# NguyenThaiHoc1/CustomKnowledgeGraphEmbedding

Measured on AMD Instinct MI355X. Metric: scored (pos+neg) triples/sec, WN18RR InterHT d=1000 n_neg=256, 1/2/4/8 GPU, higher is better.
Workload: dtype f32; 1 GPU; WN18RR InterHT d=1000 -de -tr gamma=24 n_neg=256 bz=512; global_batch=512, n_neg=256, hidden_dim=1000, score_function=InterHT, parallelism=single

## Files before the change

### customknowledgegraphembedding_amd/_lib.py

```python
from __future__ import annotations

import ctypes
import os
import threading

_HERE = os.path.dirname(os.path.abspath(__file__))
LIB_PATH = os.environ.get("KGE_HIP_LIB", os.path.join(_HERE, "libkge_hip.so"))

FN_IDS = {
    "TransE": 0,
    "DistMult": 1,
    "ComplEx": 2,
    "RotatE": 3,
    "InterHT": 4,
    "pRotatE": 5,
}
HEAD_BATCH, TAIL_BATCH, SINGLE = 0, 1, 3

_c_i64 = ctypes.c_int64
_c_f = ctypes.c_float
_c_p = ctypes.c_void_p
_c_i = ctypes.c_int


# ... 33 lines not shown
        _c_i,
        [_c_i, _c_i, _c_p, _c_i64, _c_i64, _c_p, _c_i64, _c_i64, _c_i64, _c_p, _c_p, _c_i64,
         _c_i64, _c_i64, _c_i64, _c_f, _c_f, _c_f, _c_p, _c_i64, _c_p, _c_p],
    ),
    "kge_step_forward_ex": (
        _c_i,
        [_c_i, _c_i, _c_p, _c_i64, _c_i64, _c_p, _c_i64, _c_i64, _c_i64, _c_p, _c_p, _c_i64,
         _c_i64, _c_i64, _c_i64, _c_f, _c_f, _c_f, _c_f, _c_i, _c_p, _c_i64, _c_p, _c_p, _c_p, _c_p, _c_p, _c_p],
    ),
    "kge_step_plan_size": (_c_i64, [_c_i, _c_i64, _c_i64, _c_i64, _c_i64, _c_i64, _c_i64, _c_i64, _c_i64]),
    "kge_step_plan": (
        _c_i, [_c_i, _c_i, _c_i64, _c_i64, _c_i64, _c_i64, _c_i64, _c_p, _c_p, _c_i64, _c_i64, _c_i64, _c_i64, _c_p,
               _c_p]),
    "kge_step_forward_planned": (
        _c_i,
        [_c_i, _c_i, _c_p, _c_i64, _c_i64, _c_p, _c_i64, _c_i64, _c_i64, _c_i64, _c_i64, _c_i64, _c_f, _c_f, _c_f,
         _c_f, _c_i, _c_p, _c_p, _c_p, _c_i64, _c_i, _c_p, _c_p, _c_i64, _c_p, _c_p, _c_p, _c_p],
    ),
    "kge_step_planner_create": (
        _c_i, [_c_p, _c_i, _c_p, _c_i64, _c_i64, _c_p, _c_i64, _c_i64, _c_i64, _c_i64, _c_i64, _c_i64, _c_f, _c_f, _c_f,
               _c_f, _c_i, _c_p, _c_p, _c_i64, _c_p]),
    "kge_step_planner_set_modulus": (_c_i, [_c_p, _c_f]),
    "kge_step_planner_set_sweep": (_c_i, [_c_p, _c_i]),
    "kge_step_planner_plan": (_c_i, [_c_p, _c_p, _c_p, _c_i64, _c_i]),
    "kge_step_planner_step": (_c_i, [_c_p, _c_p, _c_p, _c_i64, _c_i, _c_p, _c_p, _c_p, _c_p]),
    "kge_step_planner_destroy": (_c_i, [_c_p]),
    "kge_step_finish": (
        _c_i,
        [_c_i, _c_p, _c_i64, _c_i64, _c_p, _c_i64, _c_i64, _c_i64, _c_p, _c_i64, _c_i64,
         _c_f, _c_f, _c_f, _c_p, _c_i64, _c_i64, _c_f, _c_i, _c_p, _c_p, _c_p, _c_p],
    ),
    "kge_score_sharded": (
        _c_i,
        [_c_i, _c_i, _c_p, _c_i64, _c_p, _c_i64, _c_i64, _c_i64, _c_p, _c_i64, _c_i64, _c_i64,
         _c_p, _c_p, _c_i64, _c_i64, _c_i64, _c_i64, _c_f, _c_f, _c_f, _c_p, _c_i64, _c_p],
    ),
    "kge_gather_rows": (
        _c_i, [_c_p, _c_i64, _c_i64, _c_i64, _c_p, _c_i64, _c_i64, _c_i64, _c_p, _c_i64, _c_p]),
    "kge_build_id": (ctypes.c_char_p, []),
    "kge_source_hash": (ctypes.c_char_p, []),
    "kge_shard_plan": (
        _c_i, [_c_p, _c_p, _c_i64, _c_i64, _c_i64, _c_i64, _c_i, _c_i, _c_i, _c_i, _c_i, _c_p, _c_p, _c_p, _c_p, _c_p,
               _c_p, _c_p, _c_p]),
    "kge_shard_gather_queries": (
        _c_i, [_c_p, _c_i64, _c_i64, _c_i64, _c_p, _c_i64, _c_i, _c_i, _c_i64, _c_i, _c_i, _c_i, _c_i, _c_p, _c_p,
               _c_p, _c_p, _c_p, _c_p]),
# ... 189 lines not shown
```

### customknowledgegraphembedding_amd/csrc/kge_abi.hip

```cpp
#include <string.h>

#include <algorithm>
#include <cmath>

#include <string>

#include "kge_device.h"
#include "kge_scan.h"

namespace kge_impl {
namespace {

__global__ __launch_bounds__(kBlock) void neg_reduce_kernel(const float* __restrict__ s, int64_t B, int64_t N,
                                                            int64_t ld, float T, int adversarial,
                                                            float* __restrict__ out) {
    const int64_t b = (int64_t)blockIdx.x * kWavesPerBlock + (threadIdx.x >> 6);
    if (b >= B) return;
    const int lane = threadIdx.x & 63;
    const float res = row_reduce_fast(s + b * ld, N, T, adversarial, lane);
    if (lane == 0) out[b] = res;
}

__global__ __launch_bounds__(kBlock) void neg_rows_kernel(ScoreParams p) {
    const int64_t b = (int64_t)blockIdx.x * kWavesPerBlock + (threadIdx.x >> 6);
// ... 508 lines not shown

int step_order(int64_t nentity, int64_t N, const kge_forms* forms = nullptr) {
    const int forced = forms ? forms->step_order : -1;
    if (nentity >= (int64_t)8 << 25) return 0;
    if (forced >= 0 && forced <= 2) return forced;
    return N >= 128 ? 2 : 0;
}
bool use_xcd_order(int64_t nentity, int64_t N, const kge_forms* forms = nullptr) {
    return step_order(nentity, N, forms) != 0;
}

int tile_plan(int fn, ScoreParams& p, const kge_forms* forms = nullptr) {
    int V = 1, G = 1;
    if (pick_vg(p, V, G)) return 0;
    if (G > kFwdGradMaxG || p.N + 1 > 65536 || p.c_rows <= 0) return 0;
    const int64_t opb = (int64_t)G * kWave * V * 4;
    int64_t P2 = 0;
    if (fn == KGE_INTERHT && p.B <= kTileSortMaxB) {
        P2 = kWave;
        while (P2 < p.B) P2 <<= 1;
    }
    const int64_t row_bytes = (int64_t)p.D * 4 * (is_split(fn) ? 2 : 1);
    p.tile_waves = row_bytes >= 4096 ? 12 : 16;
    const int fw = forms ? forms->tile_waves : 0;
    if (fw == 8 || fw == 12 || fw == 16) p.tile_waves = fw;
    const int64_t NT = (int64_t)p.tile_waves * kWave;
    const int64_t qrow = tile_nq(fn) * opb + 8 + 8 + 8 + 4, lrow = (p.N + 1) * 4;
    const int64_t fixed = kTileBuckets * 4 + 16;
    const int64_t sort_ints = P2 ? (kTileSortMaxB + NT - 1) / NT * p.tile_waves * kTileSortRel : 0;
    auto lds = [&](int64_t R, int64_t QS) { return R * qrow + QS * opb + fixed + std::max(R * lrow, sort_ints * 4); };
    int64_t R = kTileMaxRows;
    if (forms && forms->tile_rows > 0) R = std::min<int64_t>(R, forms->tile_rows);
    while (R >= 1 && lds(R, 0) > kTileLdsMax) --R;
    if (R < 1) return 0;
    int64_t QS = 0;
    if (fn == KGE_INTERHT)
        while (QS < R && lds(R, QS + 1) <= kTileLdsMax) ++QS;
    if (forms && forms->tile_q2slots >= 0) QS = std::min<int64_t>(QS, forms->tile_q2slots);
#ifdef KGE_PROFILING_KNOBS
    p.tile_dry = getenv("KGE_TILE_DRY") ? std::max(1, atoi(getenv("KGE_TILE_DRY"))) : 0;
    if (getenv("KGE_TILE_NOSORT")) P2 = 0;
#endif
    p.tile_rows = (int)R;
    p.tile_q2slots = (int)QS;
    p.tile_sort = (int)P2;
    p.tile_lds = (int)lds(R, QS);
    return 1;
}

int planned_tile_params(int fn, int64_t nentity, int64_t ent_ld, int64_t nrelation, int64_t rel_ld, int64_t rel_off,
                        int64_t B, int64_t N, int64_t D, ScoreParams& p) {
    if (B <= 0 || N <= 0 || D <= 0 || nentity <= 0 || nentity >= ((int64_t)1 << 31) || B >= ((int64_t)1 << 31))
        return 0;
    const float* tab = reinterpret_cast<const float*>((uintptr_t)4096);
    fill_indexed(p, fn, KGE_TAIL_BATCH, tab, nentity, ent_ld, tab, nrelation, rel_ld, rel_off, nullptr, nullptr, 0, B,
                 N, D, 0.f, 1.f, 0.f);
    return tile_plan(fn, p) ? p.tile_rows : 0;
}

PlanArgs plan_args(const ScoreParams& tp, int mode, int64_t nentity, int64_t nrelation, const int64_t* pos,
                   const int64_t* neg, int64_t neg_ld, int64_t B, int64_t N, void* plan) {
    PlanArgs a;
    a.pos = pos;
    a.neg = neg;
    a.neg_ld = neg_ld;
    a.B = B;
    a.N = N;
    a.nent = nentity;
    a.nrel = nrelation;
    a.mode = mode;
    a.R = tp.tile_rows;
    a.sort = tp.tile_sort != 0;
    a.plan = reinterpret_cast<int*>(plan);
    return a;
}

}

int set_error(int code, const char* msg) { return fail(code, msg); }
}
// ... 135 lines not shown
        return fail(KGE_EINVAL, "kge_step_plan needs a negative mode (0 or 1)");
    if (B <= 0 || N <= 0 || D <= 0) return fail(KGE_EINVAL, "bad shape (B, N, D)");
    if (!pos || !neg || !plan) return fail(KGE_EINVAL, "null pointer");
    if (!aligned(plan, 16)) return fail(KGE_EINVAL, "the plan must be 16-B aligned");
    ScoreParams tp;
    if (!planned_tile_params(fn, nentity, ent_ld, nrelation, rel_ld, rel_off, B, N, D, tp))
        return fail(KGE_ENOTSUP, "the tile form does not apply to this shape (kge_step_plan_size is 0)");
    const PlanArgs a = plan_args(tp, mode, nentity, nrelation, pos, neg, neg_ld, B, N, plan);
    const unsigned groups = (unsigned)plan_groups(B, tp.tile_rows);
    if (tp.tile_waves == 16)
        hipLaunchKernelGGL(tile_plan_kernel<16>, dim3(groups), dim3(16 * kWave), plan_lds_ints(16 * kWave) * 4,
                           (hipStream_t)stream, a);
    else
        hipLaunchKernelGGL(tile_plan_kernel<12>, dim3(groups), dim3(12 * kWave), plan_lds_ints(12 * kWave) * 4,
                           (hipStream_t)stream, a);
    return check_launch("kge_step_plan");
}

static int step_forward_planned(int fn, int mode, const float* ent, int64_t nentity, int64_t ent_ld, const float* rel,
                                int64_t nrelation, int64_t rel_ld, int64_t rel_off, int64_t B, int64_t N, int64_t D,
                                float gamma, float emb_range, float modulus, float temperature, int adversarial,
                                const void* plan, const int64_t* next_pos, const int64_t* next_neg,
                                int64_t next_neg_ld, int next_mode, void* next_plan, float* neg_scores, int64_t ns_ld,
                                float* out_neg, float* pos_scores, float* out_pos, int reverse, void* stream);

int kge_step_forward_planned(int fn, int mode, const float* ent, int64_t nentity, int64_t ent_ld, const float* rel,
                             int64_t nrelation, int64_t rel_ld, int64_t rel_off, int64_t B, int64_t N, int64_t D,
                             float gamma, float emb_range, float modulus, float temperature, int adversarial,
                             const void* plan, const int64_t* next_pos, const int64_t* next_neg, int64_t next_neg_ld,
                             int next_mode, void* next_plan, float* neg_scores, int64_t ns_ld, float* out_neg,
                             float* pos_scores, float* out_pos, void* stream) {
    return step_forward_planned(fn, mode, ent, nentity, ent_ld, rel, nrelation, rel_ld, rel_off, B, N, D, gamma,
                                emb_range, modulus, temperature, adversarial, plan, next_pos, next_neg, next_neg_ld,
                                next_mode, next_plan, neg_scores, ns_ld, out_neg, pos_scores, out_pos, 0, stream);
}

static int step_forward_planned(int fn, int mode, const float* ent, int64_t nentity, int64_t ent_ld, const float* rel,
                                int64_t nrelation, int64_t rel_ld, int64_t rel_off, int64_t B, int64_t N, int64_t D,
                                float gamma, float emb_range, float modulus, float temperature, int adversarial,
                                const void* plan, const int64_t* next_pos, const int64_t* next_neg,
                                int64_t next_neg_ld, int next_mode, void* next_plan, float* neg_scores, int64_t ns_ld,
                                float* out_neg, float* pos_scores, float* out_pos, int reverse, void* stream) {
    int rc = check_fn_mode(fn, mode);
    if (rc) return rc;
    if (mode == KGE_SINGLE) return fail(KGE_EINVAL, "kge_step_forward_planned needs a negative mode (0 or 1)");
    if (B <= 0 || N <= 0 || D <= 0) return fail(KGE_EINVAL, "bad shape (B, N, D)");
    if (!ent || !rel || !plan || !neg_scores || !out_neg || !out_pos) return fail(KGE_EINVAL, "null pointer");
    if (next_plan) {
        if (next_mode != KGE_HEAD_BATCH && next_mode != KGE_TAIL_BATCH)
            return fail(KGE_EINVAL, "the next batch needs a negative mode (0 or 1)");
        if (!next_pos || !next_neg) return fail(KGE_EINVAL, "next_plan needs next_pos and next_neg");
        if (next_plan == plan) return fail(KGE_EINVAL, "next_plan must not be the plan this step reads");
        if (!aligned(next_plan, 16)) return fail(KGE_EINVAL, "the plan must be 16-B aligned");
    }
    if (!aligned(plan, 16)) return fail(KGE_EINVAL, "the plan must be 16-B aligned");
    ScoreParams tp;
    const int R = planned_tile_params(fn, nentity, ent_ld, nrelation, rel_ld, rel_off, B, N, D, tp);
    ScoreParams p;
    fill_indexed(p, fn, mode, ent, nentity, ent_ld, rel, nrelation, rel_ld, rel_off, nullptr, nullptr, 0, B, N, D,
                 gamma, emb_range, modulus);
    if (!R || !tile_plan(fn, p) || p.tile_rows != R)
        return fail(KGE_ENOTSUP, "the tile form does not apply to these tables (unaligned rows, or "
                                 "kge_step_plan_size is 0): use kge_step_forward");
    p.out = neg_scores;
    p.out_ld = ns_ld;
    p.pos_base = nullptr;
    p.temperature = temperature;
    p.adversarial = adversarial;
    p.out_neg = out_neg;
    p.out_pos_raw = pos_scores;
    p.out_pos_ls = out_pos;
    p.tile_pos = 1;
    p.tile_rev = reverse;
    p.tile_plan = reinterpret_cast<const int*>(plan);
    if (next_plan) {
        p.tile_next = plan_args(tp, next_mode, nentity, nrelation, next_pos, next_neg, next_neg_ld, B, N, next_plan);
        p.tile_lds = std::max(p.tile_lds, plan_lds_ints(p.tile_waves * kWave) * 4);
    }
    rc = run_score(fn, mode, p, KIND_STEP_FWD_TILE, stream);
    if (rc) return rc;
    const int64_t blocks = (B + kWavesPerBlock - 1) / kWavesPerBlock;
    hipLaunchKernelGGL(neg_rows_kernel, dim3((unsigned)blocks), dim3(kBlock), 0, (hipStream_t)stream, p);
    return check_launch("kge_step_forward_planned row reductions");
}

struct kge_step_planner {
    int fn = 0, adversarial = 1;
    const float* ent = nullptr;
    const float* rel = nullptr;
    int64_t nentity = 0, ent_ld = 0, nrelation = 0, rel_ld = 0, rel_off = 0, B = 0, N = 0, D = 0;
    float gamma = 0.f, emb_range = 0.f, modulus = 0.f, temperature = 1.f;
    void* plans[2] = {nullptr, nullptr};
    int cur = -1;
    int mode = 0;
    int sweep = 1;
    int64_t steps = 0;
    void* stream = nullptr;
};

int kge_step_planner_create(kge_step_planner** out, int fn, const float* ent, int64_t nentity, int64_t ent_ld,
                            const float* rel, int64_t nrelation, int64_t rel_ld, int64_t rel_off, int64_t B, int64_t N,
                            int64_t D, float gamma, float emb_range, float modulus, float temperature, int adversarial,
                            void* plan0, void* plan1, int64_t plan_bytes, void* stream) {
    if (!out) return fail(KGE_EINVAL, "kge_step_planner_create: null pointer");
    *out = nullptr;
    const int64_t need = kge_step_plan_size(fn, nentity, ent_ld, nrelation, rel_ld, rel_off, B, N, D);
    if (need <= 0) return fail(KGE_ENOTSUP, "kge_step_planner_create: the tile form does not apply to this shape");
    if (!ent || !rel || !plan0 || !plan1 || plan0 == plan1) return fail(KGE_EINVAL, "kge_step_planner_create: bad pointers");
    if (plan_bytes < need || !aligned(plan0, 16) || !aligned(plan1, 16))
        return fail(KGE_EINVAL, "kge_step_planner_create: plan buffers too small or not 16-B aligned");
    kge_step_planner* sp = new kge_step_planner;
    sp->fn = fn;
    sp->ent = ent;
    sp->nentity = nentity;
    sp->ent_ld = ent_ld;
    sp->rel = rel;
    sp->nrelation = nrelation;
    sp->rel_ld = rel_ld;
    sp->rel_off = rel_off;
    sp->B = B;
    sp->N = N;
    sp->D = D;
    sp->gamma = gamma;
    sp->emb_range = emb_range;
    sp->modulus = modulus;
    sp->temperature = temperature;
    sp->adversarial = adversarial;
    sp->plans[0] = plan0;
    sp->plans[1] = plan1;
    sp->stream = stream;
    *out = sp;
    return ok();
}

int kge_step_planner_set_modulus(kge_step_planner* sp, float modulus) {
    if (!sp) return fail(KGE_EINVAL, "kge_step_planner_set_modulus: null pointer");
    sp->modulus = modulus;
    return ok();
}

int kge_step_planner_set_sweep(kge_step_planner* sp, int alternate) {
    if (!sp) return fail(KGE_EINVAL, "kge_step_planner_set_sweep: null pointer");
    if (alternate != 0 && alternate != 1) return fail(KGE_EINVAL, "kge_step_planner_set_sweep: 0 or 1");
    sp->sweep = alternate;
    return ok();
}

int kge_step_planner_plan(kge_step_planner* sp, const int64_t* pos, const int64_t* neg, int64_t neg_ld, int mode) {
    if (!sp) return fail(KGE_EINVAL, "kge_step_planner_plan: null pointer");
    const int buf = sp->cur < 0 ? 0 : sp->cur;
    const int rc = kge_step_plan(sp->fn, mode, sp->nentity, sp->ent_ld, sp->nrelation, sp->rel_ld, sp->rel_off, pos, neg,
                                 neg_ld, sp->B, sp->N, sp->D, sp->plans[buf], sp->stream);
    if (rc) return rc;
    sp->cur = buf;
    sp->mode = mode;
    return ok();
}

int kge_step_planner_step(kge_step_planner* sp, const int64_t* next_pos, const int64_t* next_neg, int64_t next_neg_ld,
                          int next_mode, float* neg_scores, float* out_neg, float* pos_scores, float* out_pos) {
    if (!sp) return fail(KGE_EINVAL, "kge_step_planner_step: null pointer");
    if (sp->cur < 0) return fail(KGE_EINVAL, "kge_step_planner_step: no batch planned (kge_step_planner_plan first)");
    const bool nxt = next_pos && next_neg;
    const int rc = step_forward_planned(
        sp->fn, sp->mode, sp->ent, sp->nentity, sp->ent_ld, sp->rel, sp->nrelation, sp->rel_ld, sp->rel_off, sp->B,
        sp->N, sp->D, sp->gamma, sp->emb_range, sp->modulus, sp->temperature, sp->adversarial, sp->plans[sp->cur],
        next_pos, next_neg, next_neg_ld, next_mode, nxt ? sp->plans[1 - sp->cur] : nullptr, neg_scores, sp->N, out_neg,
        pos_scores, out_pos, sp->sweep ? (int)(sp->steps & 1) : 0, sp->stream);
    if (rc) return rc;
    ++sp->steps;
    if (nxt) {
        sp->cur = 1 - sp->cur;
        sp->mode = next_mode;
    } else {
        sp->cur = -1;
    }
    return ok();
}

int kge_step_planner_destroy(kge_step_planner* sp) {
    delete sp;
    return ok();
}

int kge_score_sharded(int fn, int mode, const float* qent, int64_t q_ld, const float* rel, int64_t nrelation,
                      int64_t rel_ld, int64_t rel_off, const float* shard, int64_t shard_rows, int64_t shard_ld,
                      int64_t shard_lo, const int64_t* pos, const int64_t* neg, int64_t neg_ld, int64_t B, int64_t N,
                      int64_t D, float gamma, float emb_range, float modulus, float* scores, int64_t scores_ld,
                      void* stream) {
    int rc = check_fn_mode(fn, mode);
    if (rc) return rc;
// ... 1028 lines not shown
```

### customknowledgegraphembedding_amd/csrc/kge_device.h

```cpp
#pragma once

#include <math.h>

#include <type_traits>

#include "kge_internal.h"

namespace kge_impl {

template <int V>
struct alignas(4 * V) vecf {
    float a[V];
};

template <int V>
__device__ __forceinline__ vecf<V> vzero() {
    vecf<V> r;
#pragma unroll
    for (int i = 0; i < V; ++i) r.a[i] = 0.f;
    return r;
}

template <int V>
__device__ __forceinline__ vecf<V> vload(const float* p, bool ok) {
// ... 881 lines not shown
    }
    auto chk = [](int64_t id, int64_t n) { return (id >= 0 && id < n) ? (int)id : -1; };
    if (t < R)
        reinterpret_cast<int4*>(a.plan + kPlanHdr)[(int64_t)g * R + t] =
            t < nr ? make_int4(brow[t], chk(ph, a.nent), chk(pr, a.nrel), chk(pt, a.nent)) : make_int4(-1, -1, -1, -1);
    if (g == 0 && t == 0) {
        int* h = a.plan;
        h[0] = kPlanMagic;
        h[1] = (int)a.B;
        h[2] = (int)a.N;
        h[3] = a.mode;
        h[4] = R;
        h[5] = (int)a.nent;
        h[6] = a.sort;
    }
}

template <int NWV>
__global__ __launch_bounds__(NWV * kWave) void tile_plan_kernel(PlanArgs a) {
    extern __shared__ __attribute__((aligned(16))) unsigned char plan_smem[];
    tile_plan_group<NWV>(a, (int)blockIdx.x, reinterpret_cast<int*>(plan_smem));
}

template <int FN, bool CH, int V, int G, int NWV>
__global__ __launch_bounds__(NWV * kWave) void step_fwd_tile_kernel(ScoreParams p) {
    extern __shared__ __attribute__((aligned(16))) unsigned char tile_smem[];
    constexpr int NQ = tile_nq(FN);
    constexpr int W = G * kWave;
    constexpr int NT = NWV * kWave;
    const int R = p.tile_rows, QS = p.tile_q2slots;
    vecf<V>* qimg = reinterpret_cast<vecf<V>*>(tile_smem);
    vecf<V>* q2img = qimg + (size_t)R * NQ * W;
    int64_t* rrow = reinterpret_cast<int64_t*>(q2img + (size_t)QS * W);
    int64_t* brow = rrow + R;
    int64_t* qid = brow + R;
    int* q2slot = reinterpret_cast<int*>(qid + R);
    int* hist = q2slot + R;
    int* cntp = hist + kTileBuckets;
    int* list = cntp + 4;
    const int t = threadIdx.x, lane = t & 63, w = t >> 6;
    if (p.tile_next.plan && (int)blockIdx.x >= p.tile_blocks) {
        tile_plan_group<NWV>(p.tile_next, (int)blockIdx.x - p.tile_blocks, reinterpret_cast<int*>(tile_smem));
        return;
    }
    const int x = (int)(blockIdx.x & 7);
    const int gi = (int)(blockIdx.x >> 3);
    const int64_t g0 = (int64_t)gi * R;
    const int nr = (int)min<int64_t>(R, p.B - g0);
// ... 233 lines not shown
        }
        if (lane == kWave - 1) cntp[0] = incl;
    }
    __syncthreads();
    if (pl) {
    } else if (in_regs) {
#pragma unroll
        for (int u = 0; u < TPI; ++u)
            if (wbk[u] >= 0) list[hist[wbk[u]] + wrk[u]] = wcd[u];
    } else {
        for (int64_t f = t; f < nf; f += NT) {
            int bk, code;
            if (item(f, bk, code)) list[atomicAdd(&hist[bk], 1)] = code;
        }
    }
    __syncthreads();
    const int cnt = pl ? pcnt : cntp[0];

    if (p.tile_dry) return;
    struct Item {
        Cand<FN, V, G> c;
        vecf<V> q2[FN == KGE_INTERHT ? G : 1];
    };
    for (int c0 = w; c0 < cnt; c0 += NT) {
        const int nc = min(kWave, (cnt - c0 + NWV - 1) / NWV);
        int code = 0;
        int64_t my_id = 0;
        if (lane < nc) {
            const int ci = p.tile_rev ? cnt - 1 - (c0 + NWV * lane) : c0 + NWV * lane;
            if (pl) {
                const int2 e = plist[plo + ci];
                code = e.y;
                my_id = e.x;
            } else {
                code = list[ci];
                const int r = code >> 16, n = code & 0xFFFF;
                const int64_t b = brow[r];
                my_id = n < p.N ? p.c_idx[b * p.c_stride + n] : p.pos_base[b * 3 + 2];
            }
        }
        auto load = [&](Item& it, int j) {
            bool ok;
            it.c.load(cand_row(p, readlane64(my_id, j), ok), ok, p.D, lane);
            if constexpr (FN == KGE_INTERHT) {
                const int r = __builtin_amdgcn_readlane(code, j) >> 16;
                const int sl = q2slot[r];
// ... 4 lines not shown
                    const int64_t ri = rrow[r];
                    const rsrc_t sr = make_rsrc(p.rel + (ri >= 0 ? ri : 0) * p.r_ld + p.r_off,
                                                ri >= 0 ? (uint32_t)p.D * 4u : 0u);
#pragma unroll
                    for (int k = 0; k < G; ++k) it.q2[k] = bload<V>(sr, goff<V>(lane, k));
                }
            }
        };
        auto score = [&](const Item& it, int j) -> float {
            const int cj = __builtin_amdgcn_readlane(code, j);
            const int r = cj >> 16, n = cj & 0xFFFF;
            const vecf<V>* qr = qimg + (size_t)r * NQ * W;
            (void)n;
            if constexpr (FN == KGE_INTERHT) {
                TileQueryIH<V, G> q{{qr, lane}, {qr + W, lane}, {}};
#pragma unroll
                for (int k = 0; k < G; ++k) q.q2[k] = it.q2[k];
                return cand_score<FN, CH, V, G>(it.c, q, p);
            } else {
                const LdsQuery<V> q{{qr, lane}, {qr + (NQ > 1 ? W : 0), lane}, {qr, lane}};
                return cand_score<FN, CH, V, G>(it.c, q, p);
            }
        };
        float my_score = 0.f;
        {
            Item x0, x1;
            load(x0, 0);
            for (int j = 0; j < nc; j += 2) {
                if (j + 1 < nc) load(x1, j + 1);
                float s = score(x0, j);
                if (lane == j) my_score = s;
                if (j + 1 < nc) {
                    if (j + 2 < nc) load(x0, j + 2);
                    s = score(x1, j + 1);
                    if (lane == j + 1) my_score = s;
                }
            }
        }
        if (lane < nc) {
            const int r = code >> 16, n = code & 0xFFFF;
            const int64_t b = brow[r];
            if (n < p.N) {
                p.out[b * p.out_ld + n] = my_score;
            } else {
                if (p.out_pos_raw) p.out_pos_raw[b] = my_score;
                p.out_pos_ls[b] = log_sigmoid(my_score);
            }
        }
    }
    if constexpr (CH) {
        if (!p.tile_pos) return;
        for (int r = w; r < nr; r += NWV) {
            const int64_t b = brow[r];
            const int4 pm = pl ? pmeta[r] : make_int4(0, 0, 0, 0);
            const int64_t tt = pl ? pm.w : p.pos_base[b * 3 + 2], row = tt - p.c_base;
            const bool valid = row >= 0 && row < p.c_rows;
            if (valid ? (row < e_lo || row >= e_hi) : x != 0) continue;
            Query<FN, false, V, G> qp;
            const int64_t hi = pl ? pm.y : p.pos_base[b * 3], rj = pl ? pm.z : p.pos_base[b * 3 + 1];
            const bool hok = hi >= 0 && hi < p.q_rows, rjok = rj >= 0 && rj < p.r_rows;
            qp.build(p.qent + (hok ? hi : 0) * p.q_ld, hok, p.rel + (rjok ? rj : 0) * p.r_ld + p.r_off, rjok, p.D,
                     lane, p);
            bool ok;
            Cand<FN, V, G> c;
            c.load(cand_row(p, tt, ok), ok, p.D, lane);
            const float s = cand_score<FN, false, V, G>(c, qp, p);
            if (lane == 0) {
                if (p.out_pos_raw) p.out_pos_raw[b] = s;
                p.out_pos_ls[b] = log_sigmoid(s);
            }
        }
    }
// ... 1763 lines not shown
                    adam_update(pp.a[i], gr.a[i], mm[h][gg].a[i], vv[h][gg].a[i], p.adam.b1, p.adam.b2, p.adam.eps,
                                p.adam.alpha, p.adam.step_size, p.adam.bc2_sqrt, p.adam.keras);
                sstore(sp, goffs[gg], pp);
                sstore(sm, goffs[gg], mm[h][gg]);
                sstore(sv, goffs[gg], vv[h][gg]);
            }
        }
        return;
    }
#pragma unroll
    for (int h = 0; h < NH; ++h) {
        const rsrc_t so = make_rsrc(p.d_out_ent + e * p.c_ld + h * D, nb);
#pragma unroll
        for (int gg = 0; gg < GW; ++gg) sstore(so, goffs[gg], h ? sb[gg] : sa[gg]);
    }
}

}

#include "kge_shard.h"

namespace kge_impl {

template <int FN, bool CH, int V, int G, int NWV>
void launch_tile(const ScoreParams& p, hipStream_t st, int blocks) {
    static const bool lds_ok = hipFuncSetAttribute(reinterpret_cast<const void*>(step_fwd_tile_kernel<FN, CH, V, G, NWV>),
                                                   hipFuncAttributeMaxDynamicSharedMemorySize, kTileLdsMax) == hipSuccess;
    (void)lds_ok;
    hipLaunchKernelGGL((step_fwd_tile_kernel<FN, CH, V, G, NWV>), dim3(blocks), dim3(NWV * kWave), p.tile_lds, st, p);
}

template <int FN, bool CH, int V, int G>
void launch_one(const ScoreParams& p, int kind, hipStream_t st, int blocks) {
    if (kind == KIND_SHARD_FWD_GRAD || kind == KIND_SHARD_POS || kind == KIND_SHARD_EPILOGUE)
        launch_shard<FN, CH, V, G>(p, kind, st, blocks);
    else if (kind == KIND_BWD)
        hipLaunchKernelGGL((score_bwd_kernel<FN, CH, V, G>), dim3(blocks), dim3(kBlock), 0, st, p);
    else if (kind == KIND_BWD_ROWS)
        hipLaunchKernelGGL((bwd_rows_kernel<FN, CH, V, G>), dim3(blocks), dim3(kBlock), 0, st, p);
    else if (kind == KIND_BWD_ENT)
        hipLaunchKernelGGL((bwd_ent_kernel<FN, CH, V, G>), dim3(blocks), dim3(kBlock), 0, st, p);
    else if (kind == KIND_BWD_STREAM) {
        if constexpr (G % kWavesPerBlock == 0)
            hipLaunchKernelGGL((bwd_stream_kernel<FN, CH, V, G>), dim3(blocks), dim3(kBlock), 0, st, p);
    } else if (kind == KIND_BWD_ENT_STREAM) {
        if constexpr (G % kWavesPerBlock == 0)
            hipLaunchKernelGGL((bwd_ent_stream_kernel<FN, CH, V, G>), dim3(blocks), dim3(kBlock), 0, st, p);
    } else if (kind == KIND_BWD_CHAIN)
        hipLaunchKernelGGL((bwd_chain_kernel<FN, CH, V, G>), dim3(blocks), dim3(kBlock), 0, st, p);
    else if (kind == KIND_FWD_STATS) {
        if constexpr (FN == KGE_INTERHT)
            hipLaunchKernelGGL((score_fwd_kernel<FN, CH, V, G, true>), dim3(blocks), dim3(kBlock), 0, st, p);
    }
    else if (kind == KIND_STEP_FWD)
        hipLaunchKernelGGL((step_fwd_kernel<FN, CH, V, G, false>), dim3(blocks), dim3(kBlock), 0, st, p);
    else if (kind == KIND_STEP_FWD_XCD)
        hipLaunchKernelGGL((step_fwd_xcd_kernel<FN, CH, V, G>), dim3(blocks), dim3(kBlock), 0, st, p);
    else if (kind == KIND_STEP_FWD_TILE || kind == KIND_SCORE_TILE) {
        if constexpr (G <= kFwdGradMaxG) {
            if (p.tile_waves == 16)
                launch_tile<FN, CH, V, G, 16>(p, st, blocks);
            else if (p.tile_waves == 12)
                launch_tile<FN, CH, V, G, 12>(p, st, blocks);
            else
                launch_tile<FN, CH, V, G, 8>(p, st, blocks);
        }
    }
    else if (kind == KIND_SCORE_SHARD_XCD)
        hipLaunchKernelGGL((score_sharded_xcd_kernel<FN, CH, V, G>), dim3(blocks), dim3(kBlock), 0, st, p);
    else if (kind == KIND_SHARD_BUCKET)
        hipLaunchKernelGGL((shard_bucket_kernel<FN, CH, V, G>), dim3(blocks), dim3(kBlock), 0, st, p);
    else if (kind == KIND_STEP_FWD_GRAD) {
        if constexpr (FN != KGE_PROTATE && G <= kFwdGradMaxG) {
            if (!p.adversarial)
                hipLaunchKernelGGL((step_fwd_grad_kernel<FN, CH, V, G, 0>), dim3(blocks), dim3(kBlock), 0, st, p);
            else if (p.detach)
                hipLaunchKernelGGL((step_fwd_grad_kernel<FN, CH, V, G, 1>), dim3(blocks), dim3(kBlock), 0, st, p);
            else
                hipLaunchKernelGGL((step_fwd_grad_kernel<FN, CH, V, G, 2>), dim3(blocks), dim3(kBlock), 0, st, p);
        }
    }
    else if (kind == KIND_STEP_EPILOGUE) {
        if constexpr (FN != KGE_PROTATE && G <= kFwdGradMaxG)
            hipLaunchKernelGGL((step_epilogue_kernel<FN, CH, V, G>), dim3(blocks), dim3(kBlock), 0, st, p);
    }
    else if (kind == KIND_STEP_FWD_STATS) {
// ... 45 lines not shown
```

### customknowledgegraphembedding_amd/csrc/kge_internal.h

```cpp
#pragma once

#include <hip/hip_runtime.h>
#include <stdint.h>

#include "kge_hip.h"

namespace kge_impl {

constexpr int kWave = 64;
constexpr int kBlock = 256;
constexpr int kWavesPerBlock = kBlock / kWave;
constexpr int kMaxG = 8;
constexpr int kBwdMaxG = 16;

enum Kind {
    KIND_FWD = 0,
    KIND_BWD = 1,
    KIND_FINISH = 2,
    KIND_BWD_ROWS = 3,
    KIND_BWD_ENT = 4,
    KIND_BWD_STREAM = 5,
    KIND_BWD_CHAIN = 6,
    KIND_FWD_STATS = 7,
    KIND_STEP_FWD = 8,
    KIND_STEP_FWD_STATS = 9,
    KIND_BWD_ENT_STREAM = 10,
    KIND_STEP_FWD_GRAD = 11,
    KIND_STEP_EPILOGUE = 12,
    KIND_SHARD_FWD_GRAD = 13,
    KIND_SHARD_POS = 14,
    KIND_SHARD_EPILOGUE = 15,
    KIND_STEP_FWD_XCD = 16,
    KIND_SCORE_SHARD_XCD = 17,
    KIND_SHARD_BUCKET = 18,
    KIND_STEP_FWD_TILE = 19,
    KIND_SCORE_TILE = 20,
};
constexpr int kTileBuckets = 256;
constexpr int kTileMaxRows = 16;
constexpr int kTileLdsMax = 160 * 1024;
constexpr int kTileSortRel = 64;
constexpr int kTileSortMaxB = 2048;
constexpr int tile_nq(int fn) { return (fn == KGE_COMPLEX || fn == KGE_ROTATE || fn == KGE_INTERHT) ? 2 : 1; }
constexpr int shard_nq(int fn) {
    return fn == KGE_INTERHT ? 3 : ((fn == KGE_COMPLEX || fn == KGE_ROTATE) ? 2 : 1);
}
constexpr int kFwdGradMaxG = 4;

constexpr int kPlanMagic = 0x4B475031;
constexpr int kPlanHdr = 16;
__host__ __device__ inline int64_t plan_groups(int64_t B, int R) { return (B + R - 1) / R; }
__host__ __device__ inline int64_t plan_soff(int64_t B, int R) { return kPlanHdr + plan_groups(B, R) * R * 4; }
__host__ __device__ inline int64_t plan_list(int64_t B, int R) { return (plan_soff(B, R) + plan_groups(B, R) * 9 + 3) & ~(int64_t)3; }
__host__ __device__ inline int64_t plan_words(int64_t B, int64_t N, int R) {
    return plan_list(B, R) + plan_groups(B, R) * R * (N + 1) * 2;
}
struct PlanArgs {
    const int64_t* pos;
    const int64_t* neg;
    int64_t neg_ld;
    int64_t B, N, nent, nrel;
    int mode;
    int R;
    int sort;
    int* plan;
};
__host__ __device__ constexpr int plan_lds_ints(int NT) {
    return kTileMaxRows + 8 * kTileBuckets + (kTileSortMaxB + NT - 1) / NT * (NT / 64) * kTileSortRel;
}

// ... 3 lines not shown
    int64_t q_ld, q_stride, q_rows;
    const float* rel;
    const int64_t* r_idx;
    int64_t r_ld, r_stride, r_rows, r_off;
    const float* cent;
    const int64_t* c_idx;
    int64_t c_ld, c_stride, c_rows, c_dense;
    int64_t c_base;
    int skip_foreign;
    const int* cmp_pre;
    const int* cmp_cnt;
    const int* cmp_tot;
    int64_t cmp_home0;
    const int2* bk_ent;
    const int* bk_start;
    int64_t bk_ld;
    int xcd_phases;
    int tile_rows;
    int tile_lds;
    int tile_pos;
    int tile_q2slots;
    int tile_sort;
    int tile_waves;
    int tile_dry;
    int tile_rev;
    const int* tile_plan;
    int tile_blocks;
    PlanArgs tile_next;
    float* out;
    int64_t out_ld;
    int64_t B, N;
    int D;
    int cpw;
    int wpr;
    float gamma;
    float phase_div;
    float modulus;
    const float* d_scores;
    int64_t d_ld;
    float* d_qent;
    float* d_rel;
    float* d_cent;
    float* d_modulus;
    const float* neg_scores;
    int64_t ns_ld, n_neg;
    float temperature;
// ... 79 lines not shown
```

### customknowledgegraphembedding_amd/ops.py

```python
from __future__ import annotations

import torch

from . import _lib
from ._lib import FN_IDS, HEAD_BATCH, SINGLE, TAIL_BATCH, check


def ctypes_ptr(t):
    return None if t is None else t.data_ptr()


def _stream(device) -> int:
    return torch.cuda.current_stream(device).cuda_stream


def _need_gpu(*ts):
    for t in ts:
        if t is not None and t.device.type != "cuda":
            raise _lib.KGEHipError(
                f"libkge_hip.so runs on ROCm devices only; got a tensor on {t.device} "
                "(there is no CPU fallback)")


def _fp32(t, name):
# ... 116 lines not shown

    def __init__(self, fn, ent, rel, rel_off, D, B, N, gamma, emb_range, modulus=0.0, temperature=1.0,
                 adversarial=True):
        import ctypes
        _need_gpu(ent, rel)
        _fp32(ent, "entity_embedding")
        _fp32(rel, "relation_embedding")
        self.fn, self.ent, self.rel, self.rel_off, self.D = fn, ent, rel, rel_off, D
        self.B, self.N = B, N
        lib = _lib.load()
        nbytes = self.plan_size(fn, ent, rel, rel_off, D, B, N)
        if nbytes <= 0:
            raise _lib.KGEHipError("kge_step_plan_size is 0: the tile form does not apply to this shape "
                                   "(use step_forward_raw)")
        self._bufs = [torch.empty(nbytes, dtype=torch.uint8, device=ent.device) for _ in range(2)]
        h = ctypes.c_void_p()
        check(lib.kge_step_planner_create(
            ctypes.addressof(h), fn, ent.data_ptr(), ent.shape[0], ent.stride(0), rel.data_ptr(), rel.shape[0],
            rel.stride(0), rel_off, B, N, D, float(gamma), float(emb_range), float(modulus), float(temperature),
            int(bool(adversarial)), self._bufs[0].data_ptr(), self._bufs[1].data_ptr(), nbytes,
            _stream(ent.device)), "kge_step_planner_create")
        self._h = h.value
        self._lib = lib
        self._step_fn = lib.kge_step_planner_step
        self._planned = False
        self._held = None
        self._pshape, self._nshape = (B, 3), (B, N)
        self._out_ok = None

    @staticmethod
    def plan_size(fn, ent, rel, rel_off, D, B, N):
        return int(_lib.load().kge_step_plan_size(fn, ent.shape[0], ent.stride(0), rel.shape[0], rel.stride(0),
                                                  rel_off, B, N, D))

    @classmethod
    def available(cls, fn, ent, rel, rel_off, D, B, N):
        return cls.plan_size(fn, ent, rel, rel_off, D, B, N) > 0

    def _check_batch(self, pos, neg, mode):
        if mode not in (HEAD_BATCH, TAIL_BATCH):
            raise ValueError("a planned step needs a negative mode (0 head-batch or 1 tail-batch)")
        if pos.shape != self._pshape or neg.shape != self._nshape:
            raise ValueError(f"a planned batch must be pos [{self.B}, 3] and neg [{self.B}, {self.N}]")
        if pos.dtype != torch.int64 or neg.dtype != torch.int64 or pos.device != self.ent.device or \
                neg.device != self.ent.device:
            raise TypeError("a planned batch must be int64 tensors on the tables' device")
        if pos.stride() != (3, 1) or neg.stride(1) != 1:
            raise ValueError("pos must be contiguous and neg row-contiguous")

    def set_sweep(self, alternate):
        check(self._lib.kge_step_planner_set_sweep(self._h, int(alternate)), "kge_step_planner_set_sweep")

    def set_modulus(self, modulus):
        check(self._lib.kge_step_planner_set_modulus(self._h, float(modulus)), "kge_step_planner_set_modulus")

    def plan(self, pos, neg, mode):
        self._check_batch(pos, neg, mode)
        check(self._lib.kge_step_planner_plan(self._h, pos.data_ptr(), neg.data_ptr(), neg.stride(0), mode),
              "kge_step_planner_plan")
        self._planned, self._held = True, (pos, neg)

    def outputs(self):
        dev = self.ent.device
        return (torch.empty((self.B,), dtype=torch.float32, device=dev),
                torch.empty((self.B,), dtype=torch.float32, device=dev),
                torch.empty((self.B, self.N), dtype=torch.float32, device=dev),
                torch.empty((self.B,), dtype=torch.float32, device=dev))

    def _check_outputs(self, out):
        if not isinstance(out, (tuple, list)) or len(out) != 4:
            raise ValueError("StepPlanner.step: out must be (out_neg, out_pos, neg_scores, pos_scores)")
        shapes = ((self.B,), (self.B,), (self.B, self.N), (self.B,))
        strides = ((1,), (1,), (self.N, 1), (1,))
        for t, shp, std, nm in zip(out, shapes, strides, ("out_neg", "out_pos", "neg_scores", "pos_scores")):
# ... 451 lines not shown
```

### include/kge_hip.h

```cpp
#ifndef KGE_HIP_H
#define KGE_HIP_H

#include <stdint.h>

#ifdef __cplusplus
extern "C" {
#endif

#define KGE_ABI_VERSION 1

enum kge_fn {
    KGE_TRANSE = 0,
    KGE_DISTMULT = 1,
    KGE_COMPLEX = 2,
    KGE_ROTATE = 3,
    KGE_INTERHT = 4,
    KGE_PROTATE = 5
};

enum kge_mode {
    KGE_HEAD_BATCH = 0,
    KGE_TAIL_BATCH = 1,
    KGE_SINGLE = 3
};
// ... 61 lines not shown
                           int64_t rel_off, int64_t B, int64_t N, int64_t D);
int kge_step_plan(int fn, int mode, int64_t nentity, int64_t ent_ld, int64_t nrelation, int64_t rel_ld,
                  int64_t rel_off, const int64_t* pos, const int64_t* neg, int64_t neg_ld, int64_t B, int64_t N,
                  int64_t D, void* plan, void* stream);
int kge_step_forward_planned(int fn, int mode,
                             const float* ent, int64_t nentity, int64_t ent_ld,
                             const float* rel, int64_t nrelation, int64_t rel_ld, int64_t rel_off,
                             int64_t B, int64_t N, int64_t D,
                             float gamma, float emb_range, float modulus,
                             float temperature, int adversarial,
                             const void* plan,
                             const int64_t* next_pos, const int64_t* next_neg, int64_t next_neg_ld, int next_mode,
                             void* next_plan,
                             float* neg_scores, int64_t ns_ld, float* out_neg,
                             float* pos_scores, float* out_pos, void* stream);

typedef struct kge_step_planner kge_step_planner;
int kge_step_planner_create(kge_step_planner** out, int fn, const float* ent, int64_t nentity, int64_t ent_ld,
                            const float* rel, int64_t nrelation, int64_t rel_ld, int64_t rel_off, int64_t B, int64_t N,
                            int64_t D, float gamma, float emb_range, float modulus, float temperature, int adversarial,
                            void* plan0, void* plan1, int64_t plan_bytes, void* stream);
int kge_step_planner_set_modulus(kge_step_planner* planner, float modulus);
int kge_step_planner_set_sweep(kge_step_planner* planner, int alternate);
int kge_step_planner_plan(kge_step_planner* planner, const int64_t* pos, const int64_t* neg, int64_t neg_ld, int mode);
int kge_step_planner_step(kge_step_planner* planner, const int64_t* next_pos, const int64_t* next_neg,
                          int64_t next_neg_ld, int next_mode, float* neg_scores, float* out_neg, float* pos_scores,
                          float* out_pos);
int kge_step_planner_destroy(kge_step_planner* planner);

int kge_step_finish(int fn,
                    const float* ent, int64_t nentity, int64_t ent_ld,
                    const float* rel, int64_t nrelation, int64_t rel_ld, int64_t rel_off,
                    const int64_t* pos, int64_t B, int64_t D,
                    float gamma, float emb_range, float modulus,
                    const float* neg_scores, int64_t N, int64_t ns_ld,
                    float temperature, int adversarial,
                    float* out_neg, float* pos_scores, float* out_pos, void* stream);

int kge_score_sharded(int fn, int mode,
                      const float* qent, int64_t q_ld,
                      const float* rel, int64_t nrelation, int64_t rel_ld, int64_t rel_off,
                      const float* shard, int64_t shard_rows, int64_t shard_ld, int64_t shard_lo,
                      const int64_t* pos, const int64_t* neg, int64_t neg_ld,
                      int64_t B, int64_t N, int64_t D,
                      float gamma, float emb_range, float modulus,
                      float* scores, int64_t scores_ld, void* stream);
// ... 275 lines not shown
```

Measured before the change: 1.505 billion triples/s.

## Add cross-block sweep throttling board and selectable candidate prefetch depth

Adds a small global "board" where each workgroup publishes which entity bucket it has reached in the sorted sweep. A group that gets more than a set lead of buckets ahead of its peers sleeps briefly, which keeps groups sweeping the entity table together so they share cache hits. For InterHT with large rows the default lead is 12 buckets, so the board is active for this workload when the group count fits the board and the CUs. It also adds a depth-1 (no prefetch) kernel variant, made the default for RotatE with large rows, plus profiling clock hooks. The cost is extra global stores and loads and possible stalls for every candidate fetched.

```diff
diff --git a/customknowledgegraphembedding_amd/_lib.py b/customknowledgegraphembedding_amd/_lib.py
--- a/customknowledgegraphembedding_amd/_lib.py
+++ b/customknowledgegraphembedding_amd/_lib.py
@@ -79,6 +79,12 @@
                _c_f, _c_i, _c_p, _c_p, _c_i64, _c_p]),
     "kge_step_planner_set_modulus": (_c_i, [_c_p, _c_f]),
     "kge_step_planner_set_sweep": (_c_i, [_c_p, _c_i]),
+    "kge_step_planner_set_form": (_c_i, [_c_p, _c_i, _c_i]),
+    "kge_step_board_size": (_c_i64, []),
+    "kge_step_planner_set_board": (_c_i, [_c_p, _c_p, _c_i64]),
+    "kge_step_planner_set_lead": (_c_i, [_c_p, _c_i]),
+    "kge_step_planner_get": (_c_i, [_c_p, _c_i]),
+    "kge_step_planner_set_clocks": (_c_i, [_c_p, _c_p, _c_i64]),
     "kge_step_planner_plan": (_c_i, [_c_p, _c_p, _c_p, _c_i64, _c_i]),
     "kge_step_planner_step": (_c_i, [_c_p, _c_p, _c_p, _c_i64, _c_i, _c_p, _c_p, _c_p, _c_p]),
     "kge_step_planner_destroy": (_c_i, [_c_p]),
diff --git a/customknowledgegraphembedding_amd/csrc/kge_abi.hip b/customknowledgegraphembedding_amd/csrc/kge_abi.hip
--- a/customknowledgegraphembedding_amd/csrc/kge_abi.hip
+++ b/customknowledgegraphembedding_amd/csrc/kge_abi.hip
@@ -554,6 +554,7 @@
     }
     const int64_t row_bytes = (int64_t)p.D * 4 * (is_split(fn) ? 2 : 1);
     p.tile_waves = row_bytes >= 4096 ? 12 : 16;
+    p.tile_depth = 2;
     const int fw = forms ? forms->tile_waves : 0;
     if (fw == 8 || fw == 12 || fw == 16) p.tile_waves = fw;
     const int64_t NT = (int64_t)p.tile_waves * kWave;
@@ -581,13 +582,28 @@
 }
 
 int planned_tile_params(int fn, int64_t nentity, int64_t ent_ld, int64_t nrelation, int64_t rel_ld, int64_t rel_off,
-                        int64_t B, int64_t N, int64_t D, ScoreParams& p) {
+                        int64_t B, int64_t N, int64_t D, ScoreParams& p, const kge_forms* forms = nullptr) {
     if (B <= 0 || N <= 0 || D <= 0 || nentity <= 0 || nentity >= ((int64_t)1 << 31) || B >= ((int64_t)1 << 31))
         return 0;
     const float* tab = reinterpret_cast<const float*>((uintptr_t)4096);
     fill_indexed(p, fn, KGE_TAIL_BATCH, tab, nentity, ent_ld, tab, nrelation, rel_ld, rel_off, nullptr, nullptr, 0, B,
                  N, D, 0.f, 1.f, 0.f);
-    return tile_plan(fn, p) ? p.tile_rows : 0;
+    return tile_plan(fn, p, forms) ? p.tile_rows : 0;
+}
+
+struct SweepForm {
+    int waves, depth, lead, tag;
+    int* board;
+    long long* clk;
+};
+
+void planned_sweep_defaults(int fn, int64_t D, int& waves, int& depth, int& lead) {
+    const int64_t row_bytes = D * 4 * (is_split(fn) ? 2 : 1);
+    waves = row_bytes >= 4096 ? 12 : 16;
+    depth = 2;
+    lead = 0;
+    if (row_bytes >= 4096 && fn == KGE_INTERHT) lead = 12;
+    if (row_bytes >= 4096 && fn == KGE_ROTATE) depth = 1;
 }
 
 PlanArgs plan_args(const ScoreParams& tp, int mode, int64_t nentity, int64_t nrelation, const int64_t* pos,
@@ -769,7 +785,8 @@
                                 float gamma, float emb_range, float modulus, float temperature, int adversarial,
                                 const void* plan, const int64_t* next_pos, const int64_t* next_neg,
                                 int64_t next_neg_ld, int next_mode, void* next_plan, float* neg_scores, int64_t ns_ld,
-                                float* out_neg, float* pos_scores, float* out_pos, int reverse, void* stream);
+                                float* out_neg, float* pos_scores, float* out_pos, int reverse, const SweepForm* sf,
+                                void* stream);
 
 int kge_step_forward_planned(int fn, int mode, const float* ent, int64_t nentity, int64_t ent_ld, const float* rel,
                              int64_t nrelation, int64_t rel_ld, int64_t rel_off, int64_t B, int64_t N, int64_t D,
@@ -779,7 +796,8 @@
                              float* pos_scores, float* out_pos, void* stream) {
     return step_forward_planned(fn, mode, ent, nentity, ent_ld, rel, nrelation, rel_ld, rel_off, B, N, D, gamma,
                                 emb_range, modulus, temperature, adversarial, plan, next_pos, next_neg, next_neg_ld,
-                                next_mode, next_plan, neg_scores, ns_ld, out_neg, pos_scores, out_pos, 0, stream);
+                                next_mode, next_plan, neg_scores, ns_ld, out_neg, pos_scores, out_pos, 0, nullptr,
+                                stream);
 }
 
 static int step_forward_planned(int fn, int mode, const float* ent, int64_t nentity, int64_t ent_ld, const float* rel,
@@ -787,7 +805,8 @@
                                 float gamma, float emb_range, float modulus, float temperature, int adversarial,
                                 const void* plan, const int64_t* next_pos, const int64_t* next_neg,
                                 int64_t next_neg_ld, int next_mode, void* next_plan, float* neg_scores, int64_t ns_ld,
-                                float* out_neg, float* pos_scores, float* out_pos, int reverse, void* stream) {
+                                float* out_neg, float* pos_scores, float* out_pos, int reverse, const SweepForm* sf,
+                                void* stream) {
     int rc = check_fn_mode(fn, mode);
     if (rc) return rc;
     if (mode == KGE_SINGLE) return fail(KGE_EINVAL, "kge_step_forward_planned needs a negative mode (0 or 1)");
@@ -806,7 +825,8 @@
     ScoreParams p;
     fill_indexed(p, fn, mode, ent, nentity, ent_ld, rel, nrelation, rel_ld, rel_off, nullptr, nullptr, 0, B, N, D,
                  gamma, emb_range, modulus);
-    if (!R || !tile_plan(fn, p) || p.tile_rows != R)
+    kge_forms fm = {-1, 0, 0, -1, sf ? sf->waves : 0, 0, 0};
+    if (!R || !tile_plan(fn, p, &fm) || p.tile_rows != R)
         return fail(KGE_ENOTSUP, "the tile form does not apply to these tables (unaligned rows, or "
                                  "kge_step_plan_size is 0): use kge_step_forward");
     p.out = neg_scores;
@@ -820,6 +840,13 @@
     p.tile_pos = 1;
     p.tile_rev = reverse;
     p.tile_plan = reinterpret_cast<const int*>(plan);
+    if (sf) {
+        p.tile_depth = sf->depth;
+        p.tile_board = sf->board;
+        p.tile_tag = sf->tag;
+        p.tile_lead = sf->lead;
+        p.tile_clk = sf->clk;
+    }
     if (next_plan) {
         p.tile_next = plan_args(tp, next_mode, nentity, nrelation, next_pos, next_neg, next_neg_ld, B, N, next_plan);
         p.tile_lds = std::max(p.tile_lds, plan_lds_ints(p.tile_waves * kWave) * 4);
@@ -841,9 +868,26 @@
     int cur = -1;
     int mode = 0;
     int sweep = 1;
+    int waves = 0, depth = 0, lead = -1;
+    int* board = nullptr;
+    long long* clk = nullptr;
+    int cus = 0;
+    int64_t groups = 0;
     int64_t steps = 0;
     void* stream = nullptr;
 };
+
+static SweepForm planner_form(const kge_step_planner* sp) {
+    SweepForm f = {0, 0, 0, 0, nullptr, sp->clk};
+    planned_sweep_defaults(sp->fn, sp->D, f.waves, f.depth, f.lead);
+    if (sp->waves) f.waves = sp->waves;
+    if (sp->depth) f.depth = sp->depth;
+    if (f.waves == 8) f.depth = 2;
+    if (sp->lead >= 0) f.lead = sp->lead;
+    f.tag = (int)(sp->steps % kSweepTagMask) + 1;
+    if (sp->board && f.lead > 0 && sp->groups <= kSweepBoardLine && sp->groups * 8 <= sp->cus) f.board = sp->board;
+    return f;
+}
 
 int kge_step_planner_create(kge_step_planner** out, int fn, const float* ent, int64_t nentity, int64_t ent_ld,
                             const float* rel, int64_t nrelation, int64_t rel_ld, int64_t rel_off, int64_t B, int64_t N,
@@ -876,8 +920,77 @@
     sp->plans[0] = plan0;
     sp->plans[1] = plan1;
     sp->stream = stream;
+    ScoreParams tp;
+    sp->groups = plan_groups(B, planned_tile_params(fn, nentity, ent_ld, nrelation, rel_ld, rel_off, B, N, D, tp));
+    int dev = 0;
+    if (hipGetDevice(&dev) != hipSuccess ||
+        hipDeviceGetAttribute(&sp->cus, hipDeviceAttributeMultiprocessorCount, dev) != hipSuccess)
+        sp->cus = 0;
     *out = sp;
     return ok();
+}
+
+int kge_step_planner_set_form(kge_step_planner* sp, int waves, int depth) {
+    if (!sp) return fail(KGE_EINVAL, "kge_step_planner_set_form: null pointer");
+    if ((waves != 0 && waves != 8 && waves != 12 && waves != 16) || depth < 0 || depth > 2 || (waves == 8 && depth == 1))
+        return fail(KGE_EINVAL, "kge_step_planner_set_form: waves 0, 8, 12 or 16; depth 0, 1 or 2 (8 waves: not 1)");
+    if (waves) {
+        ScoreParams tp, tw;
+        kge_forms fm = {-1, 0, 0, -1, waves, 0, 0};
+        if (planned_tile_params(sp->fn, sp->nentity, sp->ent_ld, sp->nrelation, sp->rel_ld, sp->rel_off, sp->B, sp->N, sp->D,
+                                tw, &fm) !=
+            planned_tile_params(sp->fn, sp->nentity, sp->ent_ld, sp->nrelation, sp->rel_ld, sp->rel_off, sp->B, sp->N, sp->D,
+                                tp))
+            return fail(KGE_ENOTSUP, "kge_step_planner_set_form: this wave count changes the rows per group");
+    }
+    sp->waves = waves;
+    sp->depth = depth;
+    return ok();
+}
+
+int64_t kge_step_board_size(void) { return (int64_t)kSweepBoardInts * 4; }
+
+int kge_step_planner_set_board(kge_step_planner* sp, void* board, int64_t board_bytes) {
+    if (!sp) return fail(KGE_EINVAL, "kge_step_planner_set_board: null pointer");
+    if (board && (board_bytes < kge_step_board_size() || !aligned(board, 4)))
+        return fail(KGE_EINVAL, "kge_step_planner_set_board: kge_step_board_size bytes, 4-B aligned");
+    sp->board = reinterpret_cast<int*>(board);
+    return ok();
+}
+
+int kge_step_planner_set_lead(kge_step_planner* sp, int lead) {
+    if (!sp) return fail(KGE_EINVAL, "kge_step_planner_set_lead: null pointer");
+    if (lead < -1 || lead >= kTileBuckets) return fail(KGE_EINVAL, "kge_step_planner_set_lead: -1, 0 or 1..255 buckets");
+    sp->lead = lead;
+    return ok();
+}
+
+int kge_step_planner_get(const kge_step_planner* sp, int what) {
+    if (!sp) return -1;
+    const SweepForm f = planner_form(sp);
+    switch (what) {
+        case KGE_PLANNER_WAVES: return f.waves;
+        case KGE_PLANNER_DEPTH: return f.depth;
+        case KGE_PLANNER_LEAD: return f.lead;
+        case KGE_PLANNER_THROTTLE: return f.board != nullptr;
+        case KGE_PLANNER_TAG: return f.tag;
+        default: return -1;
+    }
+}
+
+int kge_step_planner_set_clocks(kge_step_planner* sp, void* clocks, int64_t clocks_bytes) {
+#ifdef KGE_PROFILING_KNOBS
+    if (!sp) return fail(KGE_EINVAL, "kge_step_planner_set_clocks: null pointer");
+    if (clocks && (clocks_bytes < sp->groups * 8 * kSweepClkMarks * 8 || !aligned(clocks, 8)))
+        return fail(KGE_EINVAL, "kge_step_planner_set_clocks: 8 * groups * 48 bytes, 8-B aligned");
+    sp->clk = reinterpret_cast<long long*>(clocks);
+    return ok();
+#else
+    (void)sp;
+    (void)clocks;
+    (void)clocks_bytes;
+    return fail(KGE_ENOTSUP, "kge_step_planner_set_clocks: a -DKGE_PROFILING_KNOBS build only");
+#endif
 }
 
 int kge_step_planner_set_modulus(kge_step_planner* sp, float modulus) {
@@ -909,11 +1022,12 @@
     if (!sp) return fail(KGE_EINVAL, "kge_step_planner_step: null pointer");
     if (sp->cur < 0) return fail(KGE_EINVAL, "kge_step_planner_step: no batch planned (kge_step_planner_plan first)");
     const bool nxt = next_pos && next_neg;
+    const SweepForm sf = planner_form(sp);
     const int rc = step_forward_planned(
         sp->fn, sp->mode, sp->ent, sp->nentity, sp->ent_ld, sp->rel, sp->nrelation, sp->rel_ld, sp->rel_off, sp->B,
         sp->N, sp->D, sp->gamma, sp->emb_range, sp->modulus, sp->temperature, sp->adversarial, sp->plans[sp->cur],
         next_pos, next_neg, next_neg_ld, next_mode, nxt ? sp->plans[1 - sp->cur] : nullptr, neg_scores, sp->N, out_neg,
-        pos_scores, out_pos, sp->sweep ? (int)(sp->steps & 1) : 0, sp->stream);
+        pos_scores, out_pos, sp->sweep ? (int)(sp->steps & 1) : 0, &sf, sp->stream);
     if (rc) return rc;
     ++sp->steps;
     if (nxt) {
diff --git a/customknowledgegraphembedding_amd/csrc/kge_device.h b/customknowledgegraphembedding_amd/csrc/kge_device.h
--- a/customknowledgegraphembedding_amd/csrc/kge_device.h
+++ b/customknowledgegraphembedding_amd/csrc/kge_device.h
@@ -927,8 +927,9 @@
     tile_plan_group<NWV>(a, (int)blockIdx.x, reinterpret_cast<int*>(plan_smem));
 }
 
-template <int FN, bool CH, int V, int G, int NWV>
+template <int FN, bool CH, int V, int G, int NWV, int DEPTH>
 __global__ __launch_bounds__(NWV * kWave) void step_fwd_tile_kernel(ScoreParams p) {
+    static_assert(DEPTH == 1 || DEPTH == 2, "candidate rows in flight per wave");
     extern __shared__ __attribute__((aligned(16))) unsigned char tile_smem[];
     constexpr int NQ = tile_nq(FN);
     constexpr int W = G * kWave;
@@ -1208,6 +1209,21 @@
         Cand<FN, V, G> c;
         vecf<V> q2[FN == KGE_INTERHT ? G : 1];
     };
+    const bool has_board = pl && p.tile_board && (p.tile_blocks >> 3) <= kSweepBoardLine;
+    const rsrc_t brs = make_rsrc(has_board ? p.tile_board + x * kSweepBoardLine : nullptr, has_board ? kSweepBoardLine * 4u : 0u);
+    const uint32_t boff_ld = (uint32_t)(lane & (kSweepBoardLine - 1)) * 4u;
+    const uint32_t boff_st = t == 0 ? (uint32_t)gi * 4u : kSweepBoardLine * 4u;
+    const int btag = p.tile_tag << kSweepTagShift;
+    const bool bpeer = has_board && lane < (p.tile_blocks >> 3) && lane != gi;
+    int bv = 0;
+#ifdef KGE_PROFILING_KNOBS
+    long long* const clk = (pl && p.tile_clk && w == 0) ? p.tile_clk + ((int64_t)x * (p.tile_blocks >> 3) + gi) * kSweepClkMarks : nullptr;
+    int cmark = 0;
+    if (clk && lane == 0) {
+        clk[0] = wall_clock64();
+        clk[5] = __builtin_amdgcn_s_getreg((3 << 11) | 20) & 15;
+    }
+#endif
     for (int c0 = w; c0 < cnt; c0 += NT) {
         const int nc = min(kWave, (cnt - c0 + NWV - 1) / NWV);
         int code = 0;
@@ -1258,19 +1274,48 @@
                 return cand_score<FN, CH, V, G>(it.c, q, p);
             }
         };
+        const int my_bk = my_id >= e_lo ? max(0, min(kTileBuckets - 1, (int)((float)(int)(my_id - e_lo) * bscale))) : 0;
+        const int my_prog = p.tile_rev ? kTileBuckets - 1 - my_bk : my_bk;
+        auto fetch = [&](Item& it, int j) {
+            const int own = __builtin_amdgcn_readlane(my_prog, j);
+            if (has_board) {
+                const bool led = bpeer && (bv & ~kSweepDone) == btag && (bv & kSweepDone) + p.tile_lead < own;
+                if (__ballot(led)) __builtin_amdgcn_s_sleep(kSweepNap);
+                vecf<1> pub;
+                pub.a[0] = __int_as_float(btag | own);
+                bstore<1>(brs, boff_st, pub);
+                bv = (int)__builtin_amdgcn_raw_buffer_load_b32(brs, boff_ld, 0, kAuxSC1);
+            }
+#ifdef KGE_PROFILING_KNOBS
+            if (clk) {
+                while (cmark < 3 && own >= 64 * (cmark + 1)) {
+                    ++cmark;
+                    if (lane == 0) clk[cmark] = wall_clock64();
+                }
+            }
+#endif
+            load(it, j);
+        };
         float my_score = 0.f;
-        {
+        if constexpr (DEPTH == 2) {
             Item x0, x1;
-            load(x0, 0);
+            fetch(x0, 0);
             for (int j = 0; j < nc; j += 2) {
-                if (j + 1 < nc) load(x1, j + 1);
+                if (j + 1 < nc) fetch(x1, j + 1);
                 float s = score(x0, j);
                 if (lane == j) my_score = s;
                 if (j + 1 < nc) {
-                    if (j + 2 < nc) load(x0, j + 2);
+                    if (j + 2 < nc) fetch(x0, j + 2);
                     s = score(x1, j + 1);
                     if (lane == j + 1) my_score = s;
                 }
+            }
+        } else {
+            Item x0;
+            for (int j = 0; j < nc; ++j) {
+                fetch(x0, j);
+                const float s = score(x0, j);
+                if (lane == j) my_score = s;
             }
         }
         if (lane < nc) {
@@ -1284,6 +1329,14 @@
             }
         }
     }
+    if (has_board) {
+        vecf<1> pub;
+        pub.a[0] = __int_as_float(btag | kSweepDone);
+        bstore<1>(brs, boff_st, pub);
+    }
+#ifdef KGE_PROFILING_KNOBS
+    if (clk && lane == 0) clk[4] = wall_clock64();
+#endif
     if constexpr (CH) {
         if (!p.tile_pos) return;
         for (int r = w; r < nr; r += NWV) {
@@ -3093,12 +3146,14 @@
 
 namespace kge_impl {
 
-template <int FN, bool CH, int V, int G, int NWV>
+template <int FN, bool CH, int V, int G, int NWV, int DEPTH = 2>
 void launch_tile(const ScoreParams& p, hipStream_t st, int blocks) {
-    static const bool lds_ok = hipFuncSetAttribute(reinterpret_cast<const void*>(step_fwd_tile_kernel<FN, CH, V, G, NWV>),
-                                                   hipFuncAttributeMaxDynamicSharedMemorySize, kTileLdsMax) == hipSuccess;
+    static const bool lds_ok =
+        hipFuncSetAttribute(reinterpret_cast<const void*>(step_fwd_tile_kernel<FN, CH, V, G, NWV, DEPTH>),
+                            hipFuncAttributeMaxDynamicSharedMemorySize, kTileLdsMax) == hipSuccess;
     (void)lds_ok;
-    hipLaunchKernelGGL((step_fwd_tile_kernel<FN, CH, V, G, NWV>), dim3(blocks), dim3(NWV * kWave), p.tile_lds, st, p);
+    hipLaunchKernelGGL((step_fwd_tile_kernel<FN, CH, V, G, NWV, DEPTH>), dim3(blocks), dim3(NWV * kWave), p.tile_lds, st,
+                       p);
 }
 
 template <int FN, bool CH, int V, int G>
@@ -3129,10 +3184,11 @@
         hipLaunchKernelGGL((step_fwd_xcd_kernel<FN, CH, V, G>), dim3(blocks), dim3(kBlock), 0, st, p);
     else if (kind == KIND_STEP_FWD_TILE || kind == KIND_SCORE_TILE) {
         if constexpr (G <= kFwdGradMaxG) {
+            const bool d1 = p.tile_depth == 1;
             if (p.tile_waves == 16)
-                launch_tile<FN, CH, V, G, 16>(p, st, blocks);
+                d1 ? launch_tile<FN, CH, V, G, 16, 1>(p, st, blocks) : launch_tile<FN, CH, V, G, 16>(p, st, blocks);
             else if (p.tile_waves == 12)
-                launch_tile<FN, CH, V, G, 12>(p, st, blocks);
+                d1 ? launch_tile<FN, CH, V, G, 12, 1>(p, st, blocks) : launch_tile<FN, CH, V, G, 12>(p, st, blocks);
             else
                 launch_tile<FN, CH, V, G, 8>(p, st, blocks);
         }
diff --git a/customknowledgegraphembedding_amd/csrc/kge_internal.h b/customknowledgegraphembedding_amd/csrc/kge_internal.h
--- a/customknowledgegraphembedding_amd/csrc/kge_internal.h
+++ b/customknowledgegraphembedding_amd/csrc/kge_internal.h
@@ -46,6 +46,14 @@
     return fn == KGE_INTERHT ? 3 : ((fn == KGE_COMPLEX || fn == KGE_ROTATE) ? 2 : 1);
 }
 constexpr int kFwdGradMaxG = 4;
+
+constexpr int kSweepBoardLine = 32;
+constexpr int kSweepBoardInts = 8 * kSweepBoardLine;
+constexpr int kSweepTagShift = 9;
+constexpr int kSweepDone = (1 << kSweepTagShift) - 1;
+constexpr int kSweepTagMask = (1 << (31 - kSweepTagShift)) - 1;
+constexpr int kSweepNap = 8;
+constexpr int kSweepClkMarks = 6;
 
 constexpr int kPlanMagic = 0x4B475031;
 constexpr int kPlanHdr = 16;
@@ -95,6 +103,11 @@
     int tile_q2slots;
     int tile_sort;
     int tile_waves;
+    int tile_depth;
+    int* tile_board;
+    int tile_tag;
+    int tile_lead;
+    long long* tile_clk;
     int tile_dry;
     int tile_rev;
     const int* tile_plan;
diff --git a/customknowledgegraphembedding_amd/ops.py b/customknowledgegraphembedding_amd/ops.py
--- a/customknowledgegraphembedding_amd/ops.py
+++ b/customknowledgegraphembedding_amd/ops.py
@@ -162,6 +162,9 @@
             _stream(ent.device)), "kge_step_planner_create")
         self._h = h.value
         self._lib = lib
+        self.board = torch.empty(int(lib.kge_step_board_size()), dtype=torch.uint8, device=ent.device)
+        check(lib.kge_step_planner_set_board(self._h, self.board.data_ptr(), self.board.numel()),
+              "kge_step_planner_set_board")
         self._step_fn = lib.kge_step_planner_step
         self._planned = False
         self._held = None
@@ -190,6 +193,16 @@
 
     def set_sweep(self, alternate):
         check(self._lib.kge_step_planner_set_sweep(self._h, int(alternate)), "kge_step_planner_set_sweep")
+
+    def set_form(self, waves=0, depth=0):
+        check(self._lib.kge_step_planner_set_form(self._h, int(waves), int(depth)), "kge_step_planner_set_form")
+
+    def set_lead(self, lead):
+        check(self._lib.kge_step_planner_set_lead(self._h, int(lead)), "kge_step_planner_set_lead")
+
+    def form(self):
+        return {k: int(self._lib.kge_step_planner_get(self._h, i))
+                for i, k in enumerate(("waves", "depth", "lead", "throttle", "tag"))}
 
     def set_modulus(self, modulus):
         check(self._lib.kge_step_planner_set_modulus(self._h, float(modulus)), "kge_step_planner_set_modulus")
diff --git a/include/kge_hip.h b/include/kge_hip.h
--- a/include/kge_hip.h
+++ b/include/kge_hip.h
@@ -107,6 +107,17 @@
                             void* plan0, void* plan1, int64_t plan_bytes, void* stream);
 int kge_step_planner_set_modulus(kge_step_planner* planner, float modulus);
 int kge_step_planner_set_sweep(kge_step_planner* planner, int alternate);
+int kge_step_planner_set_form(kge_step_planner* planner, int waves, int depth);
+int64_t kge_step_board_size(void);
+int kge_step_planner_set_board(kge_step_planner* planner, void* board, int64_t board_bytes);
+int kge_step_planner_set_lead(kge_step_planner* planner, int lead);
+#define KGE_PLANNER_WAVES 0
+#define KGE_PLANNER_DEPTH 1
+#define KGE_PLANNER_LEAD 2
+#define KGE_PLANNER_THROTTLE 3
+#define KGE_PLANNER_TAG 4
+int kge_step_planner_get(const kge_step_planner* planner, int what);
+int kge_step_planner_set_clocks(kge_step_planner* planner, void* clocks, int64_t clocks_bytes);
 int kge_step_planner_plan(kge_step_planner* planner, const int64_t* pos, const int64_t* neg, int64_t neg_ld, int mode);
 int kge_step_planner_step(kge_step_planner* planner, const int64_t* next_pos, const int64_t* next_neg,
                           int64_t next_neg_ld, int next_mode, float* neg_scores, float* out_neg, float* pos_scores,
```

Measured after the change: 1.567 billion triples/s (median of 6 runs). +4.1%, better.
